# ZechengLi19/CIM

Hardware: NVIDIA B200
Metric: CIM-head images/s (ROIAlign fwd+bwd + mask IoU + scoring fwd+bwd + mining + losses incl. PCL) (higher is better)
Workload: dtype f32

## Files before the change

cim_b200/csrc/roi_align.cu:

```cuda
#include "common.cuh"
#include <algorithm>

namespace {

constexpr int PH = 7, PW = 7, NBIN = 49;
template <bool WIDE>
struct DescL {
    static constexpr int MT = WIDE ? 12 : 8;
    static constexpr int WYP = MT + 2;
    static constexpr int WX = WIDE ? 140 : 112;
    static constexpr int WORDS = WX + 7 * MT;
};
constexpr int MAXT = DescL<false>::MT;
constexpr int WYP = DescL<false>::WYP;
constexpr int DESC_WORDS = DescL<false>::WORDS;
constexpr int DESC_WORDS_MAX = DescL<true>::WORDS;
enum {
    D_B = 0, D_FLAGY = 1, D_FLAGX = 2, D_TX = 3, D_Y0 = 4, D_Y1 = 5, D_XINC = 6, D_OWN = 7,
    D_YLO = 8, D_YN = 16, D_XLO = 24, D_PHR = 32 , D_WY = 40 , D_WX = DescL<false>::WX
};
static_assert(D_WY + 7 * DescL<false>::WYP <= DescL<false>::WX && DescL<false>::WORDS == 168, "narrow descriptor");
static_assert(D_WY + 7 * DescL<true>::WYP <= DescL<true>::WX && (DescL<true>::WX % 4) == 0 &&
              (DescL<true>::WORDS % 4) == 0 && DescL<true>::WORDS / 4 <= 64, "wide descriptor");
constexpr int WS_HDR_BYTES = 256;
// ... 147 lines not shown
                reinterpret_cast<float *>(d)[D_WX + p * MAXT + i] = v;
            }

            if (lo2 <= prev) inc = 0;
            prev = lo2;
        }
        if (inc && !flag) {
            int g3 = 1;
            for (int p = 0; p + 3 < 7; ++p)
                if (d[D_XLO + p + 3] - d[D_XLO + p] < T) g3 = 0;
            if (g3) inc = 3;
        }
        d[D_XINC] = inc;
        d[D_XLO + 7] = 0;
    }
}

__device__ __forceinline__ int tile_off(int y, int x, int W) { return (((y >> 1) * W + x) << 1) + (y & 1); }

__device__ __forceinline__ void load_tile(float *tile, const float *__restrict__ src, int H, int W,
                                          int pitch, int tid, int nthr) {
    const int HW = H * W;
    if ((W & 3) == 0) {
        const float4 *s4 = reinterpret_cast<const float4 *>(src);
        const int n4 = CH * HW / 4;
        for (int e = tid; e < n4; e += nthr) {
            const float4 v = __ldg(s4 + e);
            const int idx = e * 4, c = idx / HW, rem = idx - c * HW, y = rem / W, x = rem - y * W;
            float *dst = tile + c * pitch + tile_off(y, x, W);
            dst[0] = v.x; dst[2] = v.y; dst[4] = v.z; dst[6] = v.w;
        }
    } else {
        for (int e = tid; e < CH * HW; e += nthr) {
            const int c = e / HW, rem = e - c * HW, y = rem / W, x = rem - y * W;
            tile[c * pitch + tile_off(y, x, W)] = __ldg(src + e);
        }
    }
    if (H & 1)
        for (int e = tid; e < CH * W; e += nthr) {
            const int c = e / W, x = e - c * W;
            tile[c * pitch + tile_off(H, x, W)] = 0.f;
        }
}

__device__ __forceinline__ void cp_async16(void *smem_dst, const void *gmem_src) {
    asm volatile("cp.async.cg.shared.global [%0], [%1], 16;" ::"r"(smem_u32(smem_dst)), "l"(gmem_src) : "memory");
}
__device__ __forceinline__ void cp_async_commit() { asm volatile("cp.async.commit_group;" ::: "memory"); }
template <int N>
__device__ __forceinline__ void cp_async_wait() { asm volatile("cp.async.wait_group %0;" ::"n"(N) : "memory"); }

__device__ __forceinline__ float2 bcast2(float w) { return make_float2(w, w); }

template <int T, bool GLB>
__device__ __forceinline__ void fwd_pairs(const float *__restrict__ tile_c, int W, int xs_rt, const int *__restrict__ d,
                                          float *__restrict__ stage_c, const float4 *__restrict__ wyd, int lane) {
    const int xs = GLB ? xs_rt : 1;
    constexpr bool WREG = T <= 4;
    constexpr int TR = WREG ? T : 1;
    constexpr int MAXT = DescL<GLB>::MT;
    float wx[PW][TR];
    int xo[PW];
    const float *dwx = reinterpret_cast<const float *>(d + DescL<GLB>::WX);
    {
        int4 a = *reinterpret_cast<const int4 *>(d + D_XLO), b = *reinterpret_cast<const int4 *>(d + D_XLO + 4);
        xo[0] = a.x; xo[1] = a.y; xo[2] = a.z; xo[3] = a.w; xo[4] = b.x; xo[5] = b.y; xo[6] = b.z;
    }
    if (WREG) {
#pragma unroll
        for (int pw = 0; pw < PW; ++pw) {
            const float4 a = *reinterpret_cast<const float4 *>(dwx + pw * MAXT);
            const float t4[4] = {a.x, a.y, a.z, a.w};
#pragma unroll
            for (int l = 0; l < TR; ++l) wx[pw][l] = t4[l];
        }
    }
    float2 acc[4][PW];
#pragma unroll
    for (int q = 0; q < 4; ++q)
#pragma unroll
        for (int pw = 0; pw < PW; ++pw) acc[q][pw] = make_float2(0.f, 0.f);

    const int p0 = d[D_Y0] >> 1, p1 = (d[D_Y1] + 1) >> 1;
    const unsigned char *phr = reinterpret_cast<const unsigned char *>(d + D_PHR);
    const float2 *tile2 = reinterpret_cast<const float2 *>(tile_c);
#pragma unroll 1
    if (GLB) {
#pragma unroll
        for (int pw = 0; pw < PW; ++pw) xo[pw] *= xs;
    }
    for (int p = p0; p < p1; ++p) {
        const float2 *row = tile2 + (size_t)p * W * xs;
        float2 r[PW];
#pragma unroll
        for (int pw = 0; pw < PW; ++pw) {
            float2 t = make_float2(0.f, 0.f);
            if (WREG) {
#pragma unroll
                for (int l = 0; l < T; ++l) t = __ffma2_rn(bcast2(wx[pw][l]), row[xo[pw] + l * xs], t);
            } else {
                const float4 a = *reinterpret_cast<const float4 *>(dwx + pw * MAXT);
                const float4 b = *reinterpret_cast<const float4 *>(dwx + pw * MAXT + 4);
                float4 c = make_float4(0.f, 0.f, 0.f, 0.f);
                if (T > 8) c = *reinterpret_cast<const float4 *>(dwx + pw * MAXT + 8);
                const float t12[12] = {a.x, a.y, a.z, a.w, b.x, b.y, b.z, b.w, c.x, c.y, c.z, c.w};
#pragma unroll
                for (int l = 0; l < T; ++l) t = __ffma2_rn(bcast2(t12[l]), row[xo[pw] + l * xs], t);
            }
            r[pw] = t;
        }
        const float4 *wq = wyd + (p - p0) * 4;
        const float4 e0 = wq[0], e1 = wq[1], o0 = wq[2], o1 = wq[3];
        const float2 we[4] = {make_float2(e0.x, e0.y), make_float2(e0.z, e0.w), make_float2(e1.x, e1.y),
                              make_float2(e1.z, e1.w)};
        const float2 wo[4] = {make_float2(o0.x, o0.y), make_float2(o0.z, o0.w), make_float2(o1.x, o1.y),
                              make_float2(o1.z, o1.w)};
        const int code = phr[p - p0];
        const int qlo = (code & 15) >> 1, qhi = ((code & 15) + (code >> 4) - 1) >> 1;
#pragma unroll
        for (int q = 0; q < 4; ++q)
            if (q >= qlo && q <= qhi) {
#pragma unroll
                for (int pw = 0; pw < PW; ++pw) {
                    acc[q][pw] = __ffma2_rn(bcast2(r[pw].x), we[q], acc[q][pw]);
                    acc[q][pw] = __ffma2_rn(bcast2(r[pw].y), wo[q], acc[q][pw]);
                }
            }
    }
    if (elect_one()) bulk_wait_read<0>();
    __syncwarp();
#pragma unroll
    for (int q = 0; q < 4; ++q)
#pragma unroll
        for (int pw = 0; pw < PW; ++pw) {
            stage_c[(2 * q) * PW + pw] = acc[q][pw].x;
            if (q < 3) stage_c[(2 * q + 1) * PW + pw] = acc[q][pw].y;
        }
}

template <bool WIDE>
__device__ __forceinline__ void build_wyd(float *wyd, const int *__restrict__ d, int lane) {
    constexpr int MAXT = DescL<WIDE>::MT, WYP = DescL<WIDE>::WYP;
    const int p0 = d[D_Y0] >> 1, np = ((d[D_Y1] + 1) >> 1) - p0;
    float4 *w4 = reinterpret_cast<float4 *>(wyd);
    for (int i = lane; i < np * 4; i += 32) w4[i] = make_float4(0.f, 0.f, 0.f, 0.f);
    __syncwarp();
    const float *dwy = reinterpret_cast<const float *>(d + D_WY);
    for (int t = lane; t < PH * MAXT; t += 32) {
        const int ph = t / MAXT, i = t - ph * MAXT;
        if (i < d[D_YN + ph]) {
            const int y = d[D_YLO + ph] + i;
            wyd[(y - 2 * p0) * 8 + ph] = dwy[ph * WYP + 1 + i];
        }
    }
    __syncwarp();
}

constexpr int FWD_MAX_WARPS = 11;

constexpr int FWD_GLOB_WARPS = 8;
template <bool GLB>
__global__ void __launch_bounds__((GLB ? FWD_GLOB_WARPS : FWD_MAX_WARPS) * 32, 1)
roi_align_fwd_tile_kernel(const float *__restrict__ feat, const int *__restrict__ hdr,
                          const int *__restrict__ img_start, const int *__restrict__ descs,
                          const float *__restrict__ mask7, float *__restrict__ out, int B, int C, int H, int W,
                          int pitch, int wyd_floats) {
    constexpr int FWD_DESC_WORDS = DescL<GLB>::WORDS;
    extern __shared__ __align__(128) float smem[];
    const int nw = blockDim.x >> 5;
    float *tile = smem;
    float *stage = smem + (GLB ? 0 : (size_t)CH * pitch);
    int *dslots = reinterpret_cast<int *>(stage + (size_t)nw * STAGE_FLOATS);
    float *wyds = reinterpret_cast<float *>(dslots + (size_t)nw * 2 * FWD_DESC_WORDS);
    __shared__ int s_next;
    if (__ldg(hdr) != 0) return;

    const int tid = threadIdx.x, lane = tid & 31, warp = tid >> 5;
    const int nchunks = C / CH;
    const size_t HW = (size_t)H * W;
    const int s0 = __ldg(img_start), sB = __ldg(img_start + B);
    const long long U = (long long)nchunks * (sB - s0);
    long long u = U * blockIdx.x / gridDim.x;
    const long long u_end = U * (blockIdx.x + 1) / gridDim.x;
    float *stage_w = stage + warp * STAGE_FLOATS;
    float *stage_c = stage_w + lane * NBIN;
    int *my_slots = dslots + warp * 2 * FWD_DESC_WORDS;
    float *my_wyd = wyds + (size_t)warp * wyd_floats;

    auto prefetch = [&](int roi, int slot) {
        const int *src = descs + (size_t)roi * FWD_DESC_WORDS;
        int *dst = my_slots + slot * FWD_DESC_WORDS;
        cp_async16(dst + lane * 4, src + lane * 4);
        if (lane < FWD_DESC_WORDS / 4 - 32) cp_async16(dst + (32 + lane) * 4, src + (32 + lane) * 4);
        cp_async_commit();
    };

    int b = 0;
    while (u < u_end) {
        while (b < B && (long long)nchunks * (__ldg(img_start + b + 1) - s0) <= u) ++b;
        const int is = __ldg(img_start + b), nroi = __ldg(img_start + b + 1) - is;
        const long long base = (long long)nchunks * (is - s0);
        const int ch = (int)((u - base) / nroi);
        const int r0 = (int)((u - base) - (long long)ch * nroi);
        const int r1 = (int)min((long long)nroi, r0 + (u_end - u));
        const int c0 = ch * CH;

        int r = r0 + warp, slot = 0;
        if (r < r1) prefetch(is + r, 0);
        const float *tile_c;
        if (GLB) {
            tile_c = feat + (((size_t)b * ((H + 1) >> 1) * W) * C + c0 + lane) * 2;
        } else {
            __syncthreads();
            if (tid == 0) s_next = r0 + nw;
            load_tile(tile, feat + ((size_t)b * C + c0) * HW, H, W, pitch, tid, blockDim.x);
            __syncthreads();
            tile_c = tile + lane * pitch;
        }
        while (r < r1) {
            int rn = r + nw;
            if (!GLB) {
                if (lane == 0) rn = atomicAdd(&s_next, 1);
                rn = __shfl_sync(0xffffffffu, rn, 0);
            }
            if (rn < r1) { prefetch(is + rn, slot ^ 1); cp_async_wait<1>(); } else { cp_async_wait<0>(); }
            __syncwarp();
            const int *d = my_slots + slot * FWD_DESC_WORDS;
            const int roi = is + r;
            if ((d[D_FLAGY] | d[D_FLAGX]) == 0) {
                build_wyd<GLB>(my_wyd, d, lane);
                const float4 *wyd4 = reinterpret_cast<const float4 *>(my_wyd);
                switch (d[D_TX]) {
                    case 2: fwd_pairs<2, GLB>(tile_c, W, C, d, stage_c, wyd4, lane); break;
                    case 3: fwd_pairs<3, GLB>(tile_c, W, C, d, stage_c, wyd4, lane); break;
                    case 4: fwd_pairs<4, GLB>(tile_c, W, C, d, stage_c, wyd4, lane); break;
                    case 6: fwd_pairs<6, GLB>(tile_c, W, C, d, stage_c, wyd4, lane); break;
                    case 8: fwd_pairs<8, GLB>(tile_c, W, C, d, stage_c, wyd4, lane); break;
                    default: fwd_pairs<GLB ? 12 : 8, GLB>(tile_c, W, C, d, stage_c, wyd4, lane); break;
                }
                fence_proxy_async_smem();
                __syncwarp();
                const size_t orow = mask7 ? (size_t)roi * 2 * C : (size_t)roi * C;
                if (elect_one()) {
                    bulk_s2g(out + (orow + c0) * NBIN, stage_w, STAGE_FLOATS * 4);
                    bulk_commit();
                }
                if (mask7) {
                    float m[NBIN];
                    const float *mp = mask7 + (size_t)roi * NBIN;
#pragma unroll
                    for (int i = 0; i < NBIN; ++i) m[i] = __ldg(mp + i);
                    if (elect_one()) bulk_wait_read<0>();
                    __syncwarp();
#pragma unroll
                    for (int i = 0; i < NBIN; ++i) stage_c[i] *= m[i];
                    fence_proxy_async_smem();
                    __syncwarp();
                    if (elect_one()) {
                        bulk_s2g(out + (orow + C + c0) * NBIN, stage_w, STAGE_FLOATS * 4);
                        bulk_commit();
                    }
                }
            }
            __syncwarp();
            slot ^= 1;
            r = rn;
        }
        u += r1 - r0;
    }
    if (elect_one()) bulk_wait_read<0>();
}

__device__ __forceinline__ void load_window(float *tile, const float *__restrict__ src , int H, int W,
                                            int oy, int ox, int wh, int ww, int pitch, int tid, int nthr) {
    const size_t HW = (size_t)H * W;
    const int area = wh * ww;
    if (((W | ox | ww) & 3) == 0) {
        const int q = ww >> 2, n4 = CH * wh * q;
        for (int e = tid; e < n4; e += nthr) {
            const int c = e / (wh * q), rem = e - c * wh * q, y = rem / q, x = (rem - y * q) << 2;
            float4 v = make_float4(0.f, 0.f, 0.f, 0.f);
            if (oy + y < H) v = __ldg(reinterpret_cast<const float4 *>(src + c * HW + (size_t)(oy + y) * W + ox + x));
            float *dst = tile + c * pitch + tile_off(y, x, ww);
            dst[0] = v.x; dst[2] = v.y; dst[4] = v.z; dst[6] = v.w;
        }
    } else {
        for (int e = tid; e < CH * area; e += nthr) {
            const int c = e / area, rem = e - c * area, y = rem / ww, x = rem - y * ww;
            tile[c * pitch + tile_off(y, x, ww)] = oy + y < H ? __ldg(src + c * HW + (size_t)(oy + y) * W + ox + x) : 0.f;
        }
    }
}

__device__ __forceinline__ int win_find_bucket(const int *__restrict__ bucket, int lo, int hi, int s) {
    while (hi - lo > 1) {
        const int mid = (lo + hi) >> 1;
        if (__ldg(bucket + mid) <= s) lo = mid; else hi = mid;
    }
    return lo;
}

__device__ __forceinline__ void win_store_partial(float *stage_c, const int *d, float *__restrict__ out_c,
                                                  const float *__restrict__ mask, float *__restrict__ out2_c) {
    const unsigned ym = (unsigned)d[DW_YMAP], xm = (unsigned)d[DW_XMAP];
    const int ny = (ym >> 28) & 7, nx = (xm >> 28) & 7;
    for (int ys = 0; ys < ny; ++ys) {
        int first = 0;
        for (int xs = 1; xs < nx; ++xs) {
            if (((xm >> (4 * xs)) & 15u) == ((xm >> (4 * (xs - 1))) & 15u)) stage_c[ys * PW + first] += stage_c[ys * PW + xs];
            else first = xs;
        }
    }
    int firsty = 0;
    for (int ys = 1; ys < ny; ++ys) {
        if (((ym >> (4 * ys)) & 15u) == ((ym >> (4 * (ys - 1))) & 15u)) {
            for (int xs = 0; xs < nx; ++xs) stage_c[firsty * PW + xs] += stage_c[ys * PW + xs];
        } else firsty = ys;
    }
    for (int ys = 0; ys < ny; ++ys) {
        const int by = (ym >> (4 * ys)) & 15;
        if (ys > 0 && (int)((ym >> (4 * (ys - 1))) & 15u) == by) continue;
        for (int xs = 0; xs < nx; ++xs) {
            const int bx = (xm >> (4 * xs)) & 15;
// ... 17 lines not shown
    float *wyds = reinterpret_cast<float *>(dslots + (size_t)nw * 2 * DESC_WORDS);
    __shared__ int s_next;

    const int tid = threadIdx.x, lane = tid & 31, warp = tid >> 5;
    const int nchunks = C / CH, NW = g.nwy * g.nwx;
    const size_t HW = (size_t)H * W;
    const long long U = (long long)nchunks * __ldg(bucket + B * NW);
    long long u = U * blockIdx.x / gridDim.x;
    const long long u_end = U * (blockIdx.x + 1) / gridDim.x;
    float *stage_w = stage + warp * STAGE_FLOATS;
    float *stage_c = stage_w + lane * NBIN;
    int *my_slots = dslots + warp * 2 * DESC_WORDS;
    float *my_wyd = wyds + (size_t)warp * wyd_floats;

    auto prefetch = [&](int pos, int slot) {
        const int *src = descs + (size_t)pos * DESC_WORDS;
        int *dst = my_slots + slot * DESC_WORDS;
        cp_async16(dst + lane * 4, src + lane * 4);
        if (lane < DESC_WORDS / 4 - 32) cp_async16(dst + (32 + lane) * 4, src + (32 + lane) * 4);
        cp_async_commit();
    };

    int b = 0;
    while (u < u_end) {
        while (b < B && (long long)nchunks * __ldg(bucket + (b + 1) * NW) <= u) ++b;
        const int ib0 = __ldg(bucket + b * NW), nit = __ldg(bucket + (b + 1) * NW) - ib0;
        const long long base = (long long)nchunks * ib0;
        const int ch = (int)((u - base) / nit);
        const int s0 = ib0 + (int)((u - base) - (long long)ch * nit);
        const int k = win_find_bucket(bucket, b * NW, (b + 1) * NW, s0);
        const int s1 = (int)min((long long)__ldg(bucket + k + 1), s0 + (u_end - u));
        const int wy = (k - b * NW) / g.nwx, wx = (k - b * NW) - wy * g.nwx;
        const int oy = win_origin(wy, g.Hp, g.wh), ox = win_origin(wx, W, g.ww);
        const int c0 = ch * CH;

        int r = s0 + warp, slot = 0;
        if (r < s1) prefetch(r, 0);
        __syncthreads();
        if (tid == 0) s_next = s0 + nw;
        load_window(tile, feat + ((size_t)b * C + c0) * HW, H, W, oy, ox, g.wh, g.ww, pitch, tid, blockDim.x);
        __syncthreads();
        const float *tile_c = tile + lane * pitch;
        while (r < s1) {
            int rn = 0;
            if (lane == 0) rn = atomicAdd(&s_next, 1);
            rn = __shfl_sync(0xffffffffu, rn, 0);
            if (rn < s1) { prefetch(rn, slot ^ 1); cp_async_wait<1>(); } else { cp_async_wait<0>(); }
            __syncwarp();
            const int *d = my_slots + slot * DESC_WORDS;
            const int roi = d[DW_ROI];
            build_wyd<false>(my_wyd, d, lane);
            const float4 *wyd4 = reinterpret_cast<const float4 *>(my_wyd);
            switch (d[D_TX]) {
                case 2: fwd_pairs<2, false>(tile_c, g.ww, C, d, stage_c, wyd4, lane); break;
                case 3: fwd_pairs<3, false>(tile_c, g.ww, C, d, stage_c, wyd4, lane); break;
                case 4: fwd_pairs<4, false>(tile_c, g.ww, C, d, stage_c, wyd4, lane); break;
                case 6: fwd_pairs<6, false>(tile_c, g.ww, C, d, stage_c, wyd4, lane); break;
                default: fwd_pairs<8, false>(tile_c, g.ww, C, d, stage_c, wyd4, lane); break;
            }
            const size_t orow = mask7 ? (size_t)roi * 2 * C : (size_t)roi * C;
            if (d[DW_FLAGS] & 1) {
                fence_proxy_async_smem();
                __syncwarp();
                if (elect_one()) {
                    bulk_s2g(out + (orow + c0) * NBIN, stage_w, STAGE_FLOATS * 4);
                    bulk_commit();
                }
                if (mask7) {
                    float m[NBIN];
                    const float *mp = mask7 + (size_t)roi * NBIN;
#pragma unroll
                    for (int i = 0; i < NBIN; ++i) m[i] = __ldg(mp + i);
                    if (elect_one()) bulk_wait_read<0>();
                    __syncwarp();
#pragma unroll
                    for (int i = 0; i < NBIN; ++i) stage_c[i] *= m[i];
                    fence_proxy_async_smem();
                    __syncwarp();
                    if (elect_one()) {
                        bulk_s2g(out + (orow + C + c0) * NBIN, stage_w, STAGE_FLOATS * 4);
                        bulk_commit();
                    }
                }
            } else {
                win_store_partial(stage_c, d, out + (orow + c0 + lane) * NBIN,
                                  mask7 ? mask7 + (size_t)roi * NBIN : nullptr, out + (orow + C + c0 + lane) * NBIN);
            }
            __syncwarp();
            slot ^= 1;
            r = rn;
        }
        u += s1 - s0;
    }
    if (elect_one()) bulk_wait_read<0>();
}

constexpr int WIN_TM_PAD = 8;
constexpr int NWB_DEFAULT = 16;
constexpr int NBR = 4;
constexpr int NS = 3;
constexpr int NS_TM_EXTRA = -1;
constexpr int NBR_TM_MUL = 4;
constexpr int SLOT_FLOATS = NBR * (STAGE_FLOATS + DESC_WORDS);
constexpr int MASK_PAD = 52;
constexpr int NBR_F = 2, NS_F = 3;
constexpr int SLOT_FLOATS_F = NBR_F * (2 * STAGE_FLOATS + DESC_WORDS + MASK_PAD);

__device__ __forceinline__ float2 tm_ld2(uint32_t taddr) {
    uint32_t a, b;
    asm volatile("tcgen05.ld.sync.aligned.32x32b.x2.b32 {%0, %1}, [%2];" : "=r"(a), "=r"(b) : "r"(taddr) : "memory");
    return make_float2(__uint_as_float(a), __uint_as_float(b));
// ... 897 lines not shown
        const size_t oidx = mask7 ? (size_t)k * 2 * per_roi + e : (size_t)k * per_roi + e;
        const float mk = mask7 ? __ldg(mask7 + (size_t)k * oh * ow + ph * ow + pw) : 0.f;
        if (!valid_b) {
            if (!BWD) { outp[oidx] = 0.f; if (mask7) outp[oidx + per_roi] = 0.f; }
            continue;
        }
        const size_t plane = ((size_t)g.b * C + c) * H * W;
        float acc = 0.f;
        float top = BWD ? in[oidx] : 0.f;
        if (BWD && mask7) top = fmaf(in[oidx + per_roi], mk, top);
        for (int iy = 0; iy < g.gh; ++iy) {
            const float y = sample_coord(g.ys, g.bh, ph, iy, g.gh);
            for (int ix = 0; ix < g.gw; ++ix) {
                const float x = sample_coord(g.xs, g.bw, pw, ix, g.gw);
                int y0, y1, x0, x1; float a, b2, c2, d2;
                if (!corners(H, W, y, x, y0, y1, x0, x1, a, b2, c2, d2)) continue;
                if (BWD) {
                    float *p = outp + plane;
                    atomicAdd(p + y0 * W + x0, top * a / g.count);
                    atomicAdd(p + y0 * W + x1, top * b2 / g.count);
                    atomicAdd(p + y1 * W + x0, top * c2 / g.count);
                    atomicAdd(p + y1 * W + x1, top * d2 / g.count);
                } else {
                    const float *p = in + plane;
                    acc += a * __ldg(p + y0 * W + x0) + b2 * __ldg(p + y0 * W + x1) +
                           c2 * __ldg(p + y1 * W + x0) + d2 * __ldg(p + y1 * W + x1);
                }
            }
        }
        if (!BWD) {
            const float v = acc / g.count;
            outp[oidx] = v;
            if (mask7) outp[oidx + per_roi] = v * mk;
        }
    }
    }
}

__global__ void roi_mask_pad_kernel(const float *__restrict__ m, float *__restrict__ out, int K, int n) {
    const int i = blockIdx.x * blockDim.x + threadIdx.x;
    if (i >= K * MASK_PAD) return;
    const int k = i / MASK_PAD, j = i - k * MASK_PAD;
    out[i] = j < n ? m[(size_t)k * n + j] : 0.f;
}

struct Plan {
    bool tile, glob;
    bool win;
    WinGeom wg;
    int win_pitch, win_wyd_floats, win_fwd_warps, win_seg_cap;
    size_t smem_fwd_win;
    bool bwd_tm;
    size_t smem_bwd_tm, smem_bwd_fused_tm;
    int pitch, fwd_warps, wyd_floats, glob_bwd_warps, glob_bwd_warps_fused;
    size_t smem_fwd, smem_bwd, smem_bwd_fused, smem_fwd_glob, smem_bwd_glob, smem_bwd_glob_fused;
};
static Plan make_plan(int C, int H, int W, int oh, int ow) {
    Plan p{};
    const int Hp = (H + 1) & ~1, words = Hp * W;
    p.pitch = ((words >> 1) & 1) ? words : words + 2;
    p.wyd_floats = (Hp / 2) * 16;
    const size_t cap = (size_t)cim_max_smem_optin();
    const size_t per_warp = (size_t)STAGE_FLOATS * 4 + 2 * DESC_WORDS * 4 + (size_t)p.wyd_floats * 4;
    const size_t per_warp_wide = per_warp + 2 * (DESC_WORDS_MAX - DESC_WORDS) * 4;
    p.fwd_warps = FWD_MAX_WARPS;
    while (p.fwd_warps > 4 && (size_t)CH * p.pitch * 4 + p.fwd_warps * per_warp > cap) --p.fwd_warps;
    p.smem_fwd = (size_t)CH * p.pitch * 4 + p.fwd_warps * per_warp;
    p.smem_bwd = (size_t)CH * p.pitch * 4 + (size_t)NS * SLOT_FLOATS * 4 + 2 * NS * 8;
    p.smem_bwd_fused = (size_t)CH * p.pitch * 4 + (size_t)NS_F * SLOT_FLOATS_F * 4 + 2 * NS_F * 8;
    p.tile = oh == PH && ow == PW && (C % CH) == 0 && W >= MAXT && p.smem_fwd <= cap &&
             p.smem_bwd <= cap && p.smem_bwd_fused <= cap && (((size_t)CH * p.pitch * 4) % 16 == 0);
    p.bwd_tm = p.tile && 4 * ((((H + 1) >> 1) + NWB_DEFAULT - 1) / NWB_DEFAULT) * W * 2 <= 512;
    p.smem_bwd_tm = (size_t)(NS + NS_TM_EXTRA) * NBR_TM_MUL * SLOT_FLOATS * 4 + 2 * (NS + NS_TM_EXTRA) * 8;
    p.smem_bwd_fused_tm = (size_t)(NS_F + NS_TM_EXTRA) * NBR_TM_MUL * SLOT_FLOATS_F * 4 + 2 * (NS_F + NS_TM_EXTRA) * 8;
    p.smem_fwd_glob = FWD_GLOB_WARPS * per_warp_wide;
    const size_t bw = (size_t)2 * STAGE_FLOATS * 4 + 2 * DESC_WORDS_MAX * 4, bwf = bw + (size_t)2 * STAGE_FLOATS * 4;
    p.glob_bwd_warps = BWG_MAX_WARPS;
    p.glob_bwd_warps_fused = (int)std::min<size_t>(BWG_MAX_WARPS, cap / bwf);
    p.smem_bwd_glob = p.glob_bwd_warps * bw;
    p.smem_bwd_glob_fused = p.glob_bwd_warps_fused * bwf;
    p.glob = !p.tile && oh == PH && ow == PW && (C % CH) == 0 && W >= MAXT && H <= 512 && p.smem_fwd_glob <= cap &&
             p.smem_bwd_glob <= cap && p.glob_bwd_warps_fused >= 4;
    p.wg = win_geom(H, W);
    const int wwords = p.wg.wh * p.wg.ww;
    p.win_pitch = ((wwords >> 1) & 1) ? wwords : wwords + 2;
    p.win_wyd_floats = (p.wg.wh / 2) * 16;
    const size_t per_warp_win = (size_t)STAGE_FLOATS * 4 + 2 * DESC_WORDS * 4 + (size_t)p.win_wyd_floats * 4;
    p.win_fwd_warps = FWD_MAX_WARPS;
    while (p.win_fwd_warps > 4 && (size_t)CH * p.win_pitch * 4 + p.win_fwd_warps * per_warp_win > cap) --p.win_fwd_warps;
    p.smem_fwd_win = (size_t)CH * p.win_pitch * 4 + p.win_fwd_warps * per_warp_win;
    auto seg_max = [](int L, int wl) {
        if (L <= wl) return 1;
        const int emax = L / 7 + 3, per = std::max(1, (wl - (WIN_G - 1)) / emax);
        return std::min(7, (7 + per - 1) / per);
    };
    p.win_seg_cap = std::min(16, seg_max(H, p.wg.wh) * seg_max(W, p.wg.ww));
    p.win = !p.tile && oh == PH && ow == PW && (C % CH) == 0 && W >= MAXT && H >= 2 && p.wg.nwy < (1 << WIN_KEYBITS) &&
            p.wg.nwx < (1 << WIN_KEYBITS) && p.smem_fwd_win <= cap && (((size_t)CH * p.win_pitch * 4) % 16 == 0) &&
            4 * (((p.wg.wh >> 1) + NWB_DEFAULT - 1) / NWB_DEFAULT) * (p.wg.ww + WIN_TM_PAD) * 2 <= 512;
    return p;
}

static int check_args(const void *a, const void *rois, const void *c, int B, int C, int H, int W, int K,
                      int oh, int ow, const void *ws, size_t ws_bytes) {
    if (!a || !c || (K > 0 && !rois)) return CIM_ERR_ARG;
    if (B <= 0 || C <= 0 || H <= 0 || W <= 0 || K < 0 || oh <= 0 || ow <= 0) return CIM_ERR_ARG;
    if ((long long)H * W > (1 << 24) || (long long)C * oh * ow > (1LL << 30)) return CIM_ERR_SHAPE;
    if (!ws || ws_bytes < cim_roi_align_workspace_bytes(K)) return CIM_ERR_WORKSPACE;
    if (!cim_aligned(ws, 16) || !cim_aligned(a, 16) || !cim_aligned(c, 16)) return CIM_ERR_ALIGN;
    return CIM_OK;
}

static RoiWs carve(void *ws, int B, int K) {
    RoiWs w;
    char *p = (char *)ws;
    w.hdr = (int *)p;
    w.img_start = (int *)(p + ws_img_off());
    w.desc = (int *)(p + ws_desc_off(B));
    w.maskpad = (float *)(p + ws_desc_off(4096) + (size_t)(K > 0 ? K : 0) * DESC_WORDS_MAX * 4);
    return w;
}

static int run_prep(const float *rois, int B, int H, int W, int K, int oh, int ow, float scale, int sr,
// ... 57 lines not shown
CIM_API size_t cim_roi_align_workspace_bytes_ex(int B, int C, int H, int W, int K, int oh, int ow) {
    if (B <= 0 || C <= 0 || H <= 0 || W <= 0 || oh <= 0 || ow <= 0) return cim_roi_align_workspace_bytes(K);
    const Plan p = make_plan(C, H, W, oh, ow);
    size_t extra = 0;
    if (p.glob) extra = glob_copy_bytes(B, C, H, W);
    if (p.win) extra = std::max(extra, win_ws_bytes(p, B, K));
    return extra ? ws_glob_off(K) + extra : cim_roi_align_workspace_bytes(K);
}

CIM_API size_t cim_roi_align_workspace_bytes(int K) {
    return WS_HDR_BYTES + 4097 * sizeof(int) + 64 + (size_t)(K > 0 ? K : 0) * (DESC_WORDS_MAX + MASK_PAD) * 4;
}

static int roi_fwd_impl(const float *feat, const float *rois, const float *mask7, float *out, int B, int C, int H,
                        int W, int K, int oh, int ow, float scale, int sr, int aligned, void *ws, size_t ws_bytes,
                        cim_stream_t stream, bool prepared = false) {
    if (B > 4096) return CIM_ERR_SHAPE;
    if (K == 0 && feat && B > 0 && C > 0 && H > 0 && W > 0 && oh > 0 && ow > 0) return CIM_OK;
    int rc = check_args(feat, rois, out, B, C, H, W, K, oh, ow, ws, ws_bytes);
    if (rc) return rc;
    cudaStream_t st = (cudaStream_t)stream;
    const Plan p = make_plan(C, H, W, oh, ow);
    const RoiWs w = carve(ws, B, K);
    const int per_roi = C * oh * ow;
    dim3 ggrid((unsigned)K, (unsigned)min(64, (per_roi + 255) / 256));
    if (!p.tile && use_win(p, B, K, ws_bytes)) {
        const WinWs ww = carve_win(ws, p, B, K);
        if (!prepared && (rc = run_prep_win(rois, B, H, W, K, scale, sr, aligned, w, ww, p, st))) return rc;
        cudaFuncSetAttribute(roi_align_fwd_win_kernel, cudaFuncAttributeMaxDynamicSharedMemorySize, (int)p.smem_fwd_win);
        roi_align_fwd_win_kernel<<<cim_num_sms(), p.win_fwd_warps * 32, p.smem_fwd_win, st>>>(
            feat, ww.bucket, ww.desc, mask7, out, B, C, H, W, p.wg, p.win_pitch, p.win_wyd_floats);
        if ((rc = cim_launch_status())) return rc;
        roi_align_generic_kernel<false><<<dim3((unsigned)((K + 7) / 8), 1), 256, 0, st>>>(
            feat, rois, out, w.hdr, ww.flags, mask7, 1, B, C, H, W, K, oh, ow, scale, sr, aligned, 4);
        return cim_launch_status();
    }
    const bool glob = !p.tile && p.glob && ws_bytes >= ws_glob_off(K) + glob_copy_bytes(B, C, H, W);
    if (!p.tile && !glob) {
        roi_align_generic_kernel<false><<<ggrid, 256, 0, st>>>(feat, rois, out, nullptr, nullptr, mask7, 0, B, C, H, W,
                                                               K, oh, ow, scale, sr, aligned);
        return cim_launch_status();
    }
    if (!prepared && (rc = run_prep(rois, B, H, W, K, oh, ow, scale, sr, aligned, w, glob, st))) return rc;
    const long long units = (long long)(C / CH) * K;
    const int grid = (int)min((long long)cim_num_sms(), units);
    if (glob) {
        float *featP = reinterpret_cast<float *>((char *)ws + ws_glob_off(K));
        dim3 cg((unsigned)((W + 31) / 32), (unsigned)((C + 31) / 32), (unsigned)(B * ((H + 1) >> 1)));
        nchw_to_pairs_kernel<<<cg, 256, 0, st>>>(feat, reinterpret_cast<float2 *>(featP), C, H, W);
        if ((rc = cim_launch_status())) return rc;
        cudaFuncSetAttribute(roi_align_fwd_tile_kernel<true>, cudaFuncAttributeMaxDynamicSharedMemorySize,
                             (int)p.smem_fwd_glob);
        roi_align_fwd_tile_kernel<true><<<grid, FWD_GLOB_WARPS * 32, p.smem_fwd_glob, st>>>(
            featP, w.hdr, w.img_start, w.desc, mask7, out, B, C, H, W, p.pitch, p.wyd_floats);
    } else {
        cudaFuncSetAttribute(roi_align_fwd_tile_kernel<false>, cudaFuncAttributeMaxDynamicSharedMemorySize,
                             (int)p.smem_fwd);
        roi_align_fwd_tile_kernel<false><<<grid, p.fwd_warps * 32, p.smem_fwd, st>>>(
            feat, w.hdr, w.img_start, w.desc, mask7, out, B, C, H, W, p.pitch, p.wyd_floats);
    }
    if ((rc = cim_launch_status())) return rc;
    roi_align_generic_kernel<false><<<dim3((unsigned)((K + 7) / 8), 1), 256, 0, st>>>(
        feat, rois, out, w.hdr, w.desc, mask7, 1, B, C, H, W, K, oh, ow, scale, sr, aligned,
        glob ? DESC_WORDS_MAX : DESC_WORDS);
    return cim_launch_status();
}

static int roi_bwd_impl(const float *grad_out, const float *rois, const float *mask7, float *grad_feat, int B, int C,
                        int H, int W, int K, int oh, int ow, float scale, int sr, int aligned, void *ws,
                        size_t ws_bytes, cim_stream_t stream, bool prepared = false) {
    if (B > 4096) return CIM_ERR_SHAPE;
    if (K == 0 && grad_feat && B > 0 && C > 0 && H > 0 && W > 0) {
        cudaMemsetAsync(grad_feat, 0, sizeof(float) * (size_t)B * C * H * W, (cudaStream_t)stream);
        return cim_launch_status();
    }
    int rc = check_args(grad_out, rois, grad_feat, B, C, H, W, K, oh, ow, ws, ws_bytes);
    if (rc) return rc;
    cudaStream_t st = (cudaStream_t)stream;
    const Plan p = make_plan(C, H, W, oh, ow);
    const RoiWs w = carve(ws, B, K);
    const int per_roi = C * oh * ow;
    dim3 ggrid((unsigned)max(K, 1), (unsigned)min(64, (per_roi + 255) / 256));
    if (!p.tile && use_win(p, B, K, ws_bytes)) {
        const WinWs ww = carve_win(ws, p, B, K);
        if (!prepared && (rc = run_prep_win(rois, B, H, W, K, scale, sr, aligned, w, ww, p, st))) return rc;
        cudaMemsetAsync(grad_feat, 0, sizeof(float) * (size_t)B * C * H * W, st);
        const int grid = cim_num_sms();
        if (mask7) {
            roi_mask_pad_kernel<<<(K * MASK_PAD + 255) / 256, 256, 0, st>>>(mask7, w.maskpad, K, NBIN);
            if ((rc = cim_launch_status())) return rc;
            auto kern = roi_align_bwd_tile_kernel<true, NWB_DEFAULT, true, true>;
            cudaFuncSetAttribute(kern, cudaFuncAttributeMaxDynamicSharedMemorySize, (int)p.smem_bwd_fused_tm);
            kern<<<grid, NWB_DEFAULT * 32, p.smem_bwd_fused_tm, st>>>(grad_out, w.hdr, ww.bucket, ww.desc, w.maskpad,
                                                                       grad_feat, B, C, H, W, p.win_pitch, p.wg);
        } else {
            auto kern = roi_align_bwd_tile_kernel<false, NWB_DEFAULT, true, true>;
            cudaFuncSetAttribute(kern, cudaFuncAttributeMaxDynamicSharedMemorySize, (int)p.smem_bwd_tm);
            kern<<<grid, NWB_DEFAULT * 32, p.smem_bwd_tm, st>>>(grad_out, w.hdr, ww.bucket, ww.desc, nullptr, grad_feat, B,
                                                                C, H, W, p.win_pitch, p.wg);
        }
        if ((rc = cim_launch_status())) return rc;
        roi_align_generic_kernel<true><<<dim3((unsigned)((K + 7) / 8), 1), 256, 0, st>>>(
            grad_out, rois, grad_feat, w.hdr, ww.flags, mask7, 1, B, C, H, W, K, oh, ow, scale, sr, aligned, 4);
        return cim_launch_status();
    }
    const bool glob = !p.tile && p.glob && K > 0 && ws_bytes >= ws_glob_off(K) + glob_copy_bytes(B, C, H, W);
    if ((!p.tile && !glob) || K == 0) {
        cudaMemsetAsync(grad_feat, 0, sizeof(float) * (size_t)B * C * H * W, st);
        if (K > 0)
            roi_align_generic_kernel<true><<<ggrid, 256, 0, st>>>(grad_out, rois, grad_feat, nullptr, nullptr, mask7, 0,
                                                                  B, C, H, W, K, oh, ow, scale, sr, aligned);
        return cim_launch_status();
// ... 145 lines not shown
```

Measured before the change: 2243.

## Split ROIAlign forward tile work into half-ROI units with shared staging ring

After: 2022 (median of 6 runs). 9.8% lower.

```diff
diff --git a/cim_b200/csrc/roi_align.cu b/cim_b200/csrc/roi_align.cu
--- a/cim_b200/csrc/roi_align.cu
+++ b/cim_b200/csrc/roi_align.cu
@@ -223,10 +223,13 @@
 
 __device__ __forceinline__ float2 bcast2(float w) { return make_float2(w, w); }
 
-template <int T, bool GLB>
+template <int T, bool GLB, bool SPLIT, class Mid, class Wait>
 __device__ __forceinline__ void fwd_pairs(const float *__restrict__ tile_c, int W, int xs_rt, const int *__restrict__ d,
-                                          float *__restrict__ stage_c, const float4 *__restrict__ wyd, int lane) {
+                                          float *__restrict__ stage_c, const float4 *__restrict__ wyd, int half,
+                                          Mid &&mid, Wait &&wait_stage) {
     const int xs = GLB ? xs_rt : 1;
+    constexpr int NQ = SPLIT ? 2 : 4;
+    const int qb = SPLIT ? 2 * half : 0;
     constexpr bool WREG = T <= 4;
     constexpr int TR = WREG ? T : 1;
     constexpr int MAXT = DescL<GLB>::MT;
@@ -246,13 +249,24 @@
             for (int l = 0; l < TR; ++l) wx[pw][l] = t4[l];
         }
     }
-    float2 acc[4][PW];
-#pragma unroll
-    for (int q = 0; q < 4; ++q)
+    float2 acc[NQ][PW];
+#pragma unroll
+    for (int q = 0; q < NQ; ++q)
 #pragma unroll
         for (int pw = 0; pw < PW; ++pw) acc[q][pw] = make_float2(0.f, 0.f);
 
-    const int p0 = d[D_Y0] >> 1, p1 = (d[D_Y1] + 1) >> 1;
+    const int p0 = d[D_Y0] >> 1;
+    int pa = p0, pe = (d[D_Y1] + 1) >> 1;
+    if (SPLIT) {
+        int y0 = 1 << 30, y1 = 0;
+        for (int ph = 4 * half; ph < min(4 * half + 4, PH); ++ph) {
+            const int n = d[D_YN + ph];
+            if (n > 0) { y0 = min(y0, d[D_YLO + ph]); y1 = max(y1, d[D_YLO + ph] + n); }
+        }
+        pa = y1 > 0 ? y0 >> 1 : 0;
+        pe = (y1 + 1) >> 1;
+    }
+    const int pmid = (pa + pe) >> 1;
     const unsigned char *phr = reinterpret_cast<const unsigned char *>(d + D_PHR);
     const float2 *tile2 = reinterpret_cast<const float2 *>(tile_c);
 #pragma unroll 1
@@ -260,7 +274,8 @@
 #pragma unroll
         for (int pw = 0; pw < PW; ++pw) xo[pw] *= xs;
     }
-    for (int p = p0; p < p1; ++p) {
+    for (int p = pa; p < pe; ++p) {
+        if (p == pmid) mid();
         const float2 *row = tile2 + (size_t)p * W * xs;
         float2 r[PW];
 #pragma unroll
@@ -281,15 +296,21 @@
             r[pw] = t;
         }
         const float4 *wq = wyd + (p - p0) * 4;
-        const float4 e0 = wq[0], e1 = wq[1], o0 = wq[2], o1 = wq[3];
-        const float2 we[4] = {make_float2(e0.x, e0.y), make_float2(e0.z, e0.w), make_float2(e1.x, e1.y),
-                              make_float2(e1.z, e1.w)};
-        const float2 wo[4] = {make_float2(o0.x, o0.y), make_float2(o0.z, o0.w), make_float2(o1.x, o1.y),
-                              make_float2(o1.z, o1.w)};
+        float2 we[NQ], wo[NQ];
+        {
+            const float4 e0 = wq[SPLIT ? half : 0], o0 = wq[SPLIT ? 2 + half : 2];
+            we[0] = make_float2(e0.x, e0.y); we[1] = make_float2(e0.z, e0.w);
+            wo[0] = make_float2(o0.x, o0.y); wo[1] = make_float2(o0.z, o0.w);
+            if (!SPLIT) {
+                const float4 e1 = wq[1], o1 = wq[3];
+                we[NQ - 2] = make_float2(e1.x, e1.y); we[NQ - 1] = make_float2(e1.z, e1.w);
+                wo[NQ - 2] = make_float2(o1.x, o1.y); wo[NQ - 1] = make_float2(o1.z, o1.w);
+            }
+        }
         const int code = phr[p - p0];
-        const int qlo = (code & 15) >> 1, qhi = ((code & 15) + (code >> 4) - 1) >> 1;
-#pragma unroll
-        for (int q = 0; q < 4; ++q)
+        const int qlo = ((code & 15) >> 1) - qb, qhi = (((code & 15) + (code >> 4) - 1) >> 1) - qb;
+#pragma unroll
+        for (int q = 0; q < NQ; ++q)
             if (q >= qlo && q <= qhi) {
 #pragma unroll
                 for (int pw = 0; pw < PW; ++pw) {
@@ -298,16 +319,26 @@
                 }
             }
     }
-    if (elect_one()) bulk_wait_read<0>();
-    __syncwarp();
-#pragma unroll
-    for (int q = 0; q < 4; ++q)
+    wait_stage();
+    float *st = stage_c + 2 * qb * PW;
+#pragma unroll
+    for (int q = 0; q < NQ; ++q)
 #pragma unroll
         for (int pw = 0; pw < PW; ++pw) {
-            stage_c[(2 * q) * PW + pw] = acc[q][pw].x;
-            if (q < 3) stage_c[(2 * q + 1) * PW + pw] = acc[q][pw].y;
-        }
-}
+            st[(2 * q) * PW + pw] = acc[q][pw].x;
+            if (qb + q < 3) st[(2 * q + 1) * PW + pw] = acc[q][pw].y;
+        }
+}
+
+struct OwnStage {
+    __device__ __forceinline__ void operator()() const {
+        if (elect_one()) bulk_wait_read<0>();
+        __syncwarp();
+    }
+};
+struct NoOp {
+    __device__ __forceinline__ void operator()() const {}
+};
 
 template <bool WIDE>
 __device__ __forceinline__ void build_wyd(float *wyd, const int *__restrict__ d, int lane) {
@@ -328,33 +359,63 @@
 }
 
 constexpr int FWD_MAX_WARPS = 11;
+constexpr int FWD_SPLIT_WARPS = 16;
+constexpr int FWD_MAX_STAGES = 16;
+constexpr int FWD_STATIC_SMEM = 512;
+
+__device__ __forceinline__ void store_stage(float *stage_w, float *stage_c, float *__restrict__ out,
+                                            const float *__restrict__ mask7, int roi, int C, int c0) {
+    const size_t orow = mask7 ? (size_t)roi * 2 * C : (size_t)roi * C;
+    if (elect_one()) {
+        bulk_s2g(out + (orow + c0) * NBIN, stage_w, STAGE_FLOATS * 4);
+        bulk_commit();
+    }
+    if (mask7) {
+        float m[NBIN];
+        const float *mp = mask7 + (size_t)roi * NBIN;
+#pragma unroll
+        for (int i = 0; i < NBIN; ++i) m[i] = __ldg(mp + i);
+        if (elect_one()) bulk_wait_read<0>();
+        __syncwarp();
+#pragma unroll
+        for (int i = 0; i < NBIN; ++i) stage_c[i] *= m[i];
+        fence_proxy_async_smem();
+        __syncwarp();
+        if (elect_one()) {
+            bulk_s2g(out + (orow + C + c0) * NBIN, stage_w, STAGE_FLOATS * 4);
+            bulk_commit();
+        }
+    }
+}
 
 constexpr int FWD_GLOB_WARPS = 8;
 template <bool GLB>
-__global__ void __launch_bounds__((GLB ? FWD_GLOB_WARPS : FWD_MAX_WARPS) * 32, 1)
+__global__ void __launch_bounds__((GLB ? FWD_GLOB_WARPS : FWD_SPLIT_WARPS) * 32, 1)
 roi_align_fwd_tile_kernel(const float *__restrict__ feat, const int *__restrict__ hdr,
                           const int *__restrict__ img_start, const int *__restrict__ descs,
                           const float *__restrict__ mask7, float *__restrict__ out, int B, int C, int H, int W,
-                          int pitch, int wyd_floats) {
+                          int pitch, int wyd_floats, int nst) {
     constexpr int FWD_DESC_WORDS = DescL<GLB>::WORDS;
+    constexpr int UPR = GLB ? 1 : 2;
     extern __shared__ __align__(128) float smem[];
     const int nw = blockDim.x >> 5;
+    if (GLB) nst = nw;
     float *tile = smem;
     float *stage = smem + (GLB ? 0 : (size_t)CH * pitch);
-    int *dslots = reinterpret_cast<int *>(stage + (size_t)nw * STAGE_FLOATS);
+    int *dslots = reinterpret_cast<int *>(stage + (size_t)nst * STAGE_FLOATS);
     float *wyds = reinterpret_cast<float *>(dslots + (size_t)nw * 2 * FWD_DESC_WORDS);
     __shared__ int s_next;
+    __shared__ unsigned s_arrive[FWD_MAX_STAGES], s_rel[FWD_MAX_STAGES];
     if (__ldg(hdr) != 0) return;
 
     const int tid = threadIdx.x, lane = tid & 31, warp = tid >> 5;
+    if (!GLB && tid < FWD_MAX_STAGES) { s_arrive[tid] = 0; s_rel[tid] = 0; }
     const int nchunks = C / CH;
     const size_t HW = (size_t)H * W;
     const int s0 = __ldg(img_start), sB = __ldg(img_start + B);
     const long long U = (long long)nchunks * (sB - s0);
     long long u = U * blockIdx.x / gridDim.x;
     const long long u_end = U * (blockIdx.x + 1) / gridDim.x;
-    float *stage_w = stage + warp * STAGE_FLOATS;
-    float *stage_c = stage_w + lane * NBIN;
     int *my_slots = dslots + warp * 2 * FWD_DESC_WORDS;
     float *my_wyd = wyds + (size_t)warp * wyd_floats;
 
@@ -364,6 +425,19 @@
         cp_async16(dst + lane * 4, src + lane * 4);
         if (lane < FWD_DESC_WORDS / 4 - 32) cp_async16(dst + (32 + lane) * 4, src + (32 + lane) * 4);
         cp_async_commit();
+    };
+    unsigned seq = 0;
+    int pend = -1;
+    unsigned pend_rel = 0;
+    auto release = [&]() {
+        if (pend >= 0) {
+            if (elect_one()) {
+                bulk_wait_read<0>();
+                *reinterpret_cast<volatile unsigned *>(&s_rel[pend]) = pend_rel;
+            }
+            __syncwarp();
+            pend = -1;
+        }
     };
 
     int b = 0;
@@ -376,70 +450,104 @@
         const int r1 = (int)min((long long)nroi, r0 + (u_end - u));
         const int c0 = ch * CH;
 
-        int r = r0 + warp, slot = 0;
-        if (r < r1) prefetch(is + r, 0);
+        int h = UPR * r0 + warp, slot = 0;
+        const int h1 = UPR * r1;
+        if (h < h1) prefetch(is + h / UPR, 0);
         const float *tile_c;
         if (GLB) {
             tile_c = feat + (((size_t)b * ((H + 1) >> 1) * W) * C + c0 + lane) * 2;
         } else {
             __syncthreads();
-            if (tid == 0) s_next = r0 + nw;
+            if (tid == 0) s_next = UPR * r0 + nw;
             load_tile(tile, feat + ((size_t)b * C + c0) * HW, H, W, pitch, tid, blockDim.x);
             __syncthreads();
             tile_c = tile + lane * pitch;
         }
-        while (r < r1) {
-            int rn = r + nw;
+        while (h < h1) {
+            int hn = h + nw;
             if (!GLB) {
-                if (lane == 0) rn = atomicAdd(&s_next, 1);
-                rn = __shfl_sync(0xffffffffu, rn, 0);
-            }
-            if (rn < r1) { prefetch(is + rn, slot ^ 1); cp_async_wait<1>(); } else { cp_async_wait<0>(); }
+                if (lane == 0) hn = atomicAdd(&s_next, 1);
+                hn = __shfl_sync(0xffffffffu, hn, 0);
+            }
+            if (hn < h1) { prefetch(is + hn / UPR, slot ^ 1); cp_async_wait<1>(); } else { cp_async_wait<0>(); }
             __syncwarp();
             const int *d = my_slots + slot * FWD_DESC_WORDS;
-            const int roi = is + r;
-            if ((d[D_FLAGY] | d[D_FLAGX]) == 0) {
-                build_wyd<GLB>(my_wyd, d, lane);
-                const float4 *wyd4 = reinterpret_cast<const float4 *>(my_wyd);
-                switch (d[D_TX]) {
-                    case 2: fwd_pairs<2, GLB>(tile_c, W, C, d, stage_c, wyd4, lane); break;
-                    case 3: fwd_pairs<3, GLB>(tile_c, W, C, d, stage_c, wyd4, lane); break;
-                    case 4: fwd_pairs<4, GLB>(tile_c, W, C, d, stage_c, wyd4, lane); break;
-                    case 6: fwd_pairs<6, GLB>(tile_c, W, C, d, stage_c, wyd4, lane); break;
-                    case 8: fwd_pairs<8, GLB>(tile_c, W, C, d, stage_c, wyd4, lane); break;
-                    default: fwd_pairs<GLB ? 12 : 8, GLB>(tile_c, W, C, d, stage_c, wyd4, lane); break;
-                }
-                fence_proxy_async_smem();
-                __syncwarp();
-                const size_t orow = mask7 ? (size_t)roi * 2 * C : (size_t)roi * C;
-                if (elect_one()) {
-                    bulk_s2g(out + (orow + c0) * NBIN, stage_w, STAGE_FLOATS * 4);
-                    bulk_commit();
-                }
-                if (mask7) {
-                    float m[NBIN];
-                    const float *mp = mask7 + (size_t)roi * NBIN;
-#pragma unroll
-                    for (int i = 0; i < NBIN; ++i) m[i] = __ldg(mp + i);
-                    if (elect_one()) bulk_wait_read<0>();
-                    __syncwarp();
-#pragma unroll
-                    for (int i = 0; i < NBIN; ++i) stage_c[i] *= m[i];
+            const int r = h / UPR, roi = is + r;
+            const bool ok = (d[D_FLAGY] | d[D_FLAGX]) == 0;
+            if (GLB) {
+                if (ok) {
+                    float *stage_w = stage + warp * STAGE_FLOATS, *stage_c = stage_w + lane * NBIN;
+                    build_wyd<true>(my_wyd, d, lane);
+                    const float4 *wyd4 = reinterpret_cast<const float4 *>(my_wyd);
+                    switch (d[D_TX]) {
+                        case 2: fwd_pairs<2, true, false>(tile_c, W, C, d, stage_c, wyd4, 0, NoOp{}, OwnStage{}); break;
+                        case 3: fwd_pairs<3, true, false>(tile_c, W, C, d, stage_c, wyd4, 0, NoOp{}, OwnStage{}); break;
+                        case 4: fwd_pairs<4, true, false>(tile_c, W, C, d, stage_c, wyd4, 0, NoOp{}, OwnStage{}); break;
+                        case 6: fwd_pairs<6, true, false>(tile_c, W, C, d, stage_c, wyd4, 0, NoOp{}, OwnStage{}); break;
+                        case 8: fwd_pairs<8, true, false>(tile_c, W, C, d, stage_c, wyd4, 0, NoOp{}, OwnStage{}); break;
+                        default: fwd_pairs<12, true, false>(tile_c, W, C, d, stage_c, wyd4, 0, NoOp{}, OwnStage{}); break;
+                    }
                     fence_proxy_async_smem();
                     __syncwarp();
+                    store_stage(stage_w, stage_c, out, mask7, roi, C, c0);
+                }
+            } else {
+                const int half = h & 1;
+                const unsigned n = seq + (unsigned)(r - r0), use = n / (unsigned)nst;
+                const int s = (int)(n - use * (unsigned)nst);
+                float *stage_w = stage + s * STAGE_FLOATS, *stage_c = stage_w + lane * NBIN;
+                auto wait_stage = [&]() {
+                    release();
                     if (elect_one()) {
-                        bulk_s2g(out + (orow + C + c0) * NBIN, stage_w, STAGE_FLOATS * 4);
-                        bulk_commit();
+                        while (*reinterpret_cast<volatile unsigned *>(&s_rel[s]) < use) __nanosleep(20);
+                        __threadfence_block();
+                    }
+                    __syncwarp();
+                };
+                if (ok) {
+                    build_wyd<false>(my_wyd, d, lane);
+                    const float4 *wyd4 = reinterpret_cast<const float4 *>(my_wyd);
+                    switch (d[D_TX]) {
+                        case 2: fwd_pairs<2, false, true>(tile_c, W, C, d, stage_c, wyd4, half, release, wait_stage); break;
+                        case 3: fwd_pairs<3, false, true>(tile_c, W, C, d, stage_c, wyd4, half, release, wait_stage); break;
+                        case 4: fwd_pairs<4, false, true>(tile_c, W, C, d, stage_c, wyd4, half, release, wait_stage); break;
+                        case 6: fwd_pairs<6, false, true>(tile_c, W, C, d, stage_c, wyd4, half, release, wait_stage); break;
+                        default: fwd_pairs<8, false, true>(tile_c, W, C, d, stage_c, wyd4, half, release, wait_stage); break;
+                    }
+                    fence_proxy_async_smem();
+                } else {
+                    wait_stage();
+                }
+                __syncwarp();
+                unsigned last = 0;
+                if (elect_one()) {
+                    __threadfence_block();
+                    last = atomicAdd(&s_arrive[s], 1u);
+                    if (last) {
+                        s_arrive[s] = 0;
+                        __threadfence_block();
+                    }
+                }
+                if (__any_sync(0xffffffffu, last)) {
+                    if (ok) {
+                        store_stage(stage_w, stage_c, out, mask7, roi, C, c0);
+                        pend = s;
+                        pend_rel = use + 1;
+                    } else {
+                        if (elect_one()) *reinterpret_cast<volatile unsigned *>(&s_rel[s]) = use + 1;
+                        __syncwarp();
                     }
                 }
             }
             __syncwarp();
             slot ^= 1;
-            r = rn;
-        }
+            h = hn;
+        }
+        if (!GLB) release();
+        seq += (unsigned)(r1 - r0);
         u += r1 - r0;
     }
-    if (elect_one()) bulk_wait_read<0>();
+    if (GLB && elect_one()) bulk_wait_read<0>();
 }
 
 __device__ __forceinline__ void load_window(float *tile, const float *__restrict__ src , int H, int W,
@@ -563,11 +671,11 @@
             build_wyd<false>(my_wyd, d, lane);
             const float4 *wyd4 = reinterpret_cast<const float4 *>(my_wyd);
             switch (d[D_TX]) {
-                case 2: fwd_pairs<2, false>(tile_c, g.ww, C, d, stage_c, wyd4, lane); break;
-                case 3: fwd_pairs<3, false>(tile_c, g.ww, C, d, stage_c, wyd4, lane); break;
-                case 4: fwd_pairs<4, false>(tile_c, g.ww, C, d, stage_c, wyd4, lane); break;
-                case 6: fwd_pairs<6, false>(tile_c, g.ww, C, d, stage_c, wyd4, lane); break;
-                default: fwd_pairs<8, false>(tile_c, g.ww, C, d, stage_c, wyd4, lane); break;
+                case 2: fwd_pairs<2, false, false>(tile_c, g.ww, C, d, stage_c, wyd4, 0, NoOp{}, OwnStage{}); break;
+                case 3: fwd_pairs<3, false, false>(tile_c, g.ww, C, d, stage_c, wyd4, 0, NoOp{}, OwnStage{}); break;
+                case 4: fwd_pairs<4, false, false>(tile_c, g.ww, C, d, stage_c, wyd4, 0, NoOp{}, OwnStage{}); break;
+                case 6: fwd_pairs<6, false, false>(tile_c, g.ww, C, d, stage_c, wyd4, 0, NoOp{}, OwnStage{}); break;
+                default: fwd_pairs<8, false, false>(tile_c, g.ww, C, d, stage_c, wyd4, 0, NoOp{}, OwnStage{}); break;
             }
             const size_t orow = mask7 ? (size_t)roi * 2 * C : (size_t)roi * C;
             if (d[DW_FLAGS] & 1) {
@@ -1571,7 +1679,7 @@
     size_t smem_fwd_win;
     bool bwd_tm;
     size_t smem_bwd_tm, smem_bwd_fused_tm;
-    int pitch, fwd_warps, wyd_floats, glob_bwd_warps, glob_bwd_warps_fused;
+    int pitch, fwd_warps, fwd_stages, wyd_floats, glob_bwd_warps, glob_bwd_warps_fused;
     size_t smem_fwd, smem_bwd, smem_bwd_fused, smem_fwd_glob, smem_bwd_glob, smem_bwd_glob_fused;
 };
 static Plan make_plan(int C, int H, int W, int oh, int ow) {
@@ -1580,14 +1688,19 @@
     p.pitch = ((words >> 1) & 1) ? words : words + 2;
     p.wyd_floats = (Hp / 2) * 16;
     const size_t cap = (size_t)cim_max_smem_optin();
+    const size_t tile_bytes = (size_t)CH * p.pitch * 4;
     const size_t per_warp = (size_t)STAGE_FLOATS * 4 + 2 * DESC_WORDS * 4 + (size_t)p.wyd_floats * 4;
     const size_t per_warp_wide = per_warp + 2 * (DESC_WORDS_MAX - DESC_WORDS) * 4;
-    p.fwd_warps = FWD_MAX_WARPS;
-    while (p.fwd_warps > 4 && (size_t)CH * p.pitch * 4 + p.fwd_warps * per_warp > cap) --p.fwd_warps;
-    p.smem_fwd = (size_t)CH * p.pitch * 4 + p.fwd_warps * per_warp;
+    const size_t per_warp_split = per_warp - (size_t)STAGE_FLOATS * 4;
+    for (p.fwd_warps = FWD_SPLIT_WARPS;; p.fwd_warps -= 2) {
+        const size_t used = FWD_STATIC_SMEM + tile_bytes + p.fwd_warps * per_warp_split;
+        p.fwd_stages = used < cap ? (int)std::min<size_t>(FWD_MAX_STAGES, (cap - used) / (STAGE_FLOATS * 4)) : 0;
+        if (p.fwd_stages >= std::max(4, p.fwd_warps / 2) || p.fwd_warps == 4) break;
+    }
+    p.smem_fwd = tile_bytes + p.fwd_warps * per_warp_split + (size_t)p.fwd_stages * STAGE_FLOATS * 4;
     p.smem_bwd = (size_t)CH * p.pitch * 4 + (size_t)NS * SLOT_FLOATS * 4 + 2 * NS * 8;
     p.smem_bwd_fused = (size_t)CH * p.pitch * 4 + (size_t)NS_F * SLOT_FLOATS_F * 4 + 2 * NS_F * 8;
-    p.tile = oh == PH && ow == PW && (C % CH) == 0 && W >= MAXT && p.smem_fwd <= cap &&
+    p.tile = oh == PH && ow == PW && (C % CH) == 0 && W >= MAXT && p.fwd_stages >= 4 &&
              p.smem_bwd <= cap && p.smem_bwd_fused <= cap && (((size_t)CH * p.pitch * 4) % 16 == 0);
     p.bwd_tm = p.tile && 4 * ((((H + 1) >> 1) + NWB_DEFAULT - 1) / NWB_DEFAULT) * W * 2 <= 512;
     p.smem_bwd_tm = (size_t)(NS + NS_TM_EXTRA) * NBR_TM_MUL * SLOT_FLOATS * 4 + 2 * (NS + NS_TM_EXTRA) * 8;
@@ -1751,12 +1864,12 @@
         cudaFuncSetAttribute(roi_align_fwd_tile_kernel<true>, cudaFuncAttributeMaxDynamicSharedMemorySize,
                              (int)p.smem_fwd_glob);
         roi_align_fwd_tile_kernel<true><<<grid, FWD_GLOB_WARPS * 32, p.smem_fwd_glob, st>>>(
-            featP, w.hdr, w.img_start, w.desc, mask7, out, B, C, H, W, p.pitch, p.wyd_floats);
+            featP, w.hdr, w.img_start, w.desc, mask7, out, B, C, H, W, p.pitch, p.wyd_floats, 0);
     } else {
         cudaFuncSetAttribute(roi_align_fwd_tile_kernel<false>, cudaFuncAttributeMaxDynamicSharedMemorySize,
                              (int)p.smem_fwd);
         roi_align_fwd_tile_kernel<false><<<grid, p.fwd_warps * 32, p.smem_fwd, st>>>(
-            feat, w.hdr, w.img_start, w.desc, mask7, out, B, C, H, W, p.pitch, p.wyd_floats);
+            feat, w.hdr, w.img_start, w.desc, mask7, out, B, C, H, W, p.pitch, p.wyd_floats, p.fwd_stages);
     }
     if ((rc = cim_launch_status())) return rc;
     roi_align_generic_kernel<false><<<dim3((unsigned)((K + 7) / 8), 1), 256, 0, st>>>(
```
